# prachigarg23/MDIL-SS

Measured on AMD Instinct MI355X. Metric: images/sec at 1024x512 ERFNet-RA step-2 train (CS->BDD, KD on), batch 6/GPU, higher is better.
Workload: dtype f32; 1 GPU; ERFNet-RAP step-2 (2 student fwd + teacher fwd + CE + 0.1*KLD + bwd + Adam), random-init weights of the reference architecture, num_classes [20,20]; batch_per_gpu=6, global_batch=6, height=512, width=1024, parallelism=dp1

## Files before the change

### mdil_ss_amd/csrc/c16conv.hip

```cpp
#include "common.h"

namespace {

typedef unsigned int u32x4 __attribute__((ext_vector_type(4)));

constexpr int C16 = 16;
#ifndef C16_TN_
#define C16_TN_ 2
#endif
constexpr int C16_TN = C16_TN_;
constexpr int C16_PXT = 16 * C16_TN;
constexpr int C16_WAVES = 4;

struct c16_args {
  const float* in0;
  const float* in1;
  const float* wpk;
  float* out;
  mdil_epilogue e;
  int N, H, W;
  int ntaps;
  int dh[4], dw[4], src[4];
  int nwg;
};

__device__ __forceinline__ f32x4 c16_buf_load(const __amdgpu_buffer_rsrc_t r, unsigned voff) {
  const u32x4 v = __builtin_amdgcn_raw_buffer_load_b128(r, (int)voff, 0, 0);
  return __builtin_bit_cast(f32x4, v);
}

template <int NTAPS, bool EOPS>
__global__ __launch_bounds__(C16_WAVES * 64) void c16conv_kernel(const c16_args a) {
  const int lane = threadIdx.x & 63, wave = threadIdx.x >> 6;
  const int li = lane & 15, lg = lane >> 4;
  const int per = gridDim.x >> 3;
  const int g = (blockIdx.x & 7) * per + (blockIdx.x >> 3);
  if (g >= a.nwg) return;
  const int H = a.H, W = a.W, hw = H * W;
  const int npix = a.N * hw;
  const int tile = g * C16_WAVES + wave;
  const int P0 = tile * C16_PXT;
  if (P0 >= npix) return;

  const int in_bytes = npix * C16 * 4;
  const __amdgpu_buffer_rsrc_t rs0 =
      __builtin_amdgcn_make_buffer_rsrc(const_cast<float*>(a.in0), 0, in_bytes, 0x00020000);
  const __amdgpu_buffer_rsrc_t rs1 = __builtin_amdgcn_make_buffer_rsrc(
      const_cast<float*>(a.in1 ? a.in1 : a.in0), 0, in_bytes, 0x00020000);
  constexpr unsigned OOB = 0x80000000u;

  f32x4 xq[NTAPS][C16_TN];
  bool okp[C16_TN];
  long long pb[C16_TN];
#pragma unroll
  for (int n = 0; n < C16_TN; ++n) {
    const int P = P0 + 16 * n + li;
    okp[n] = P < npix;
    const int Pc = okp[n] ? P : 0;
    pb[n] = (long long)Pc * C16 + lg * 4;
    const int img = Pc / hw;
    const int rem = Pc - img * hw;
    const int h = rem / W;
    const int w = rem - h * W;
    const unsigned base = (unsigned)Pc * (unsigned)(C16 * 4) + (unsigned)lg * 16u;
#pragma unroll
    for (int t = 0; t < NTAPS; ++t) {
      const int hh = h + a.dh[t], ww = w + a.dw[t];
      const bool v = okp[n] && hh >= 0 && hh < H && ww >= 0 && ww < W;
      const unsigned voff = v ? base + (unsigned)((a.dh[t] * W + a.dw[t]) * C16 * 4) : OOB;
      xq[t][n] = c16_buf_load(a.src[t] ? rs1 : rs0, voff);
    }
  }
  const mdil_epilogue& e = a.e;
  f32x4 ra[C16_TN], rb[C16_TN];
  if constexpr (EOPS) {
    const float* opa = e.res ? e.res : e.gate;
    const float* opb = e.res_gate;
#pragma unroll
    for (int n = 0; n < C16_TN; ++n) {
      if (opa) ra[n] = *reinterpret_cast<const f32x4*>(opa + pb[n]);
      if (opb) rb[n] = *reinterpret_cast<const f32x4*>(opb + pb[n]);
    }
  }
  f32x4 wa[NTAPS];
#pragma unroll
  for (int t = 0; t < NTAPS; ++t) wa[t] = *reinterpret_cast<const f32x4*>(a.wpk + (t * C16 + li) * C16 + lg * 4);
  f32x4 vscale = {1.f, 1.f, 1.f, 1.f}, vbias = {0.f, 0.f, 0.f, 0.f};
  if (e.bias) vbias = *reinterpret_cast<const f32x4*>(e.bias + lg * 4);
  if (e.bias2) vbias += *reinterpret_cast<const f32x4*>(e.bias2 + lg * 4);
  if (e.scale) {
    vscale = *reinterpret_cast<const f32x4*>(e.scale + lg * 4);
    vbias = vbias * vscale + *reinterpret_cast<const f32x4*>(e.shift + lg * 4);
  }

  f32x4 acc[C16_TN];
#pragma unroll
  for (int n = 0; n < C16_TN; ++n) acc[n] = f32x4{0.f, 0.f, 0.f, 0.f};
#pragma unroll
  for (int t = 0; t < NTAPS; ++t)
#pragma unroll
    for (int s = 0; s < 4; ++s)
#pragma unroll
      for (int n = 0; n < C16_TN; ++n) acc[n] = mfma16(wa[t][s], xq[t][n][s], acc[n]);

#pragma unroll
  for (int n = 0; n < C16_TN; ++n) {
    f32x4 v = acc[n] * vscale + vbias;
    if (EOPS && e.res) {
      f32x4 x = ra[n];
      if (e.res_gate) {
#pragma unroll
        for (int k = 0; k < 4; ++k) x[k] = rb[n][k] > 0.f ? x[k] : 0.f;
      }
      v += x;
    }
    if (e.relu) {
#pragma unroll
      for (int k = 0; k < 4; ++k) v[k] = fmaxf(v[k], 0.f);
    }
    if (EOPS && e.gate && !e.res) {
#pragma unroll
      for (int k = 0; k < 4; ++k) v[k] = ra[n][k] > 0.f ? v[k] : 0.f;
    }
    if (okp[n]) __builtin_nontemporal_store(v, reinterpret_cast<f32x4*>(a.out + pb[n]));
  }
}

template <int NTAPS>
int launch_c16(const c16_args& a, hipStream_t st) {
  const int grid = (a.nwg + 7) / 8 * 8;
  const bool eops = a.e.res || a.e.gate || a.e.res_gate;
  if (eops)
    hipLaunchKernelGGL((c16conv_kernel<NTAPS, true>), dim3(grid), dim3(C16_WAVES * 64), 0, st, a);
  else
    hipLaunchKernelGGL((c16conv_kernel<NTAPS, false>), dim3(grid), dim3(C16_WAVES * 64), 0, st, a);
  MDIL_CHECK_LAUNCH();
  return MDIL_OK;
}

}

bool mdil_c16conv_covers(const mdil_geom* g, int cin, int cout, const mdil_epilogue* e) {
  if (cin != 16 || cout != 16 || g->ntaps != 3) return false;
  if (g->ihs != 1 || g->iws != 1 || g->ohs != 1 || g->ows != 1 || g->oho || g->owo ||
      g->HI != g->HO || g->WI != g->WO || g->OH != g->HO || g->OW != g->WO || g->out_coff ||
      g->out_pitch != 16 || g->in_pitch[0] != 16)
    return false;
  for (int t = 0; t < g->ntaps; ++t)
    if (g->src[t] && g->in_pitch[1] != 16) return false;
  if (e->res && e->gate) return false;
  return (long long)g->N * g->HO * g->WO * 16 * 4 < (1ll << 31);
}

int mdil_c16conv(const mdil_geom* g, const float* in0, const float* in1, const float* wpk,
                 const mdil_epilogue* epi, float* out, hipStream_t st) {
  c16_args a;
  memset(&a, 0, sizeof(a));
  a.in0 = in0;
  a.in1 = in1;
  a.wpk = wpk;
  a.out = out;
  a.e = *epi;
  a.N = g->N;
  a.H = g->HO;
  a.W = g->WO;
  a.ntaps = g->ntaps;
  for (int t = 0; t < g->ntaps; ++t) {
    a.dh[t] = g->dh[t];
    a.dw[t] = g->dw[t];
    a.src[t] = g->src[t];
  }
  const long long npix = (long long)g->N * g->HO * g->WO;
  const long long ntiles = (npix + C16_PXT - 1) / C16_PXT;
  a.nwg = (int)((ntiles + C16_WAVES - 1) / C16_WAVES);
  return launch_c16<3>(a, st);
}
```

### mdil_ss_amd/csrc/common.h

```cpp
#pragma once
#include <hip/hip_runtime.h>
#include <stdint.h>
#include <stdio.h>
#include <string.h>

#include "../../include/mdil_hip.h"

typedef float f32x4 __attribute__((ext_vector_type(4)));

#define MDIL_WG 256

#define MDIL_BN_MAX_BLOCKS 256

void mdil_set_error(const char* fmt, ...);

#define MDIL_CHECK_ARG(cond, ...)            \
  do {                                       \
    if (!(cond)) {                           \
      mdil_set_error(__VA_ARGS__);           \
      return MDIL_ERR_INVALID;               \
    }                                        \
  } while (0)

#define MDIL_CHECK_LAUNCH()                                              \
  do {                                                                   \
    hipError_t e__ = hipGetLastError();                                  \
    if (e__ != hipSuccess) {                                             \
      mdil_set_error("%s:%d launch failed: %s", __FILE__, __LINE__,      \
                     hipGetErrorString(e__));                            \
      return MDIL_ERR_LAUNCH;                                            \
    }                                                                    \
  } while (0)

#ifndef MDIL_HBM_PRIO
#define MDIL_HBM_PRIO 2
#endif
#define MDIL_HBM_KERNEL_PRIO() __builtin_amdgcn_s_setprio(MDIL_HBM_PRIO)

struct MdilProfScope {
  MdilProfScope(hipStream_t st, int kind, const mdil_geom* g, int cin, int cout);
  ~MdilProfScope();
  int idx;
  int path;
  hipStream_t st;
};

static inline int cdiv(long long a, long long b) { return (int)((a + b - 1) / b); }

__device__ __forceinline__ f32x4 mfma16(float a, float b, f32x4 c) {
  return __builtin_amdgcn_mfma_f32_16x16x4f32(a, b, c, 0, 0, 0);
}

__device__ __forceinline__ void welford_merge(float& n, float& mean, float& m2, float nb,
                                              float meanb, float m2b) {
  if (nb == 0.f) return;
  float nn = n + nb;
  float d = meanb - mean;
  float f = nb / nn;
  mean = mean + d * f;
  m2 = m2 + m2b + d * d * n * f;
  n = nn;
}

bool mdil_sconv_covers(const mdil_geom* g, int cin, int cout);
int mdil_sconv_stat_blocks(const mdil_geom* g, int cin);
int mdil_sconv(const mdil_geom* g, int cin, int cout, const float* in0, const float* in1,
               const float* wpk, const mdil_epilogue* epi, float* out, float* stats,
               float* stats_count, const float* bn_z, const float* bn_mean, const float* bn_invstd,
               hipStream_t st, const struct BnFinFwd* ff = nullptr, const struct BnFinBwd* fb = nullptr,
               int* fused = nullptr);

bool mdil_c16conv_covers(const mdil_geom* g, int cin, int cout, const mdil_epilogue* e);
int mdil_c16conv(const mdil_geom* g, const float* in0, const float* in1, const float* wpk,
                 const mdil_epilogue* epi, float* out, hipStream_t st);

bool mdil_wconv_covers(const mdil_geom* g, int cin, int cout);
int mdil_wconv_stat_blocks(const mdil_geom* g, int cin);
bool mdil_wconv_tail_covers(const mdil_geom* g);
struct BnFinFwd;
struct BnFinBwd;
int mdil_wconv(const mdil_geom* g, int cin, const float* in0, const float* in1, const float* wpk,
               const mdil_epilogue* epi, float* out, float* stats, float* stats_count,
               const float* bn_z, const float* bn_mean, const float* bn_invstd, hipStream_t st,
               const float* tail_gate = nullptr, const float* tail_drop = nullptr,
               const BnFinFwd* ff = nullptr, const BnFinBwd* fb = nullptr);

bool mdil_w4conv_covers(const mdil_geom* g, int cin, int cout);
int mdil_w4conv_stat_blocks(const mdil_geom* g, int cin);
int mdil_w4conv(const mdil_geom* g, int cin, const float* in0, const float* in1, const float* wpk,
                const mdil_epilogue* epi, float* out, float* stats, float* stats_count,
                const float* bn_z, const float* bn_mean, const float* bn_invstd, hipStream_t st,
                const float* tail_gate = nullptr, const float* tail_drop = nullptr,
                const BnFinFwd* ff = nullptr, const BnFinBwd* fb = nullptr);
static inline int mdil_wconv_form(const mdil_geom* g, int cin, int cout) {
  return mdil_w4conv_covers(g, cin, cout) ? 4 : mdil_wconv_covers(g, cin, cout) ? 2 : 0;
}

int mdil_bn_finalize_fwd(const float* partial, const float* pcount, int nblk, int C, const BnFinFwd& f,
                         hipStream_t st);
int mdil_bn_finalize_bwd(const float* partial, int nblk, int C, const BnFinBwd& f, hipStream_t st);
```

### mdil_ss_amd/csrc/errors.cpp

```cpp
#include <stdarg.h>
#include <stdio.h>

#include "../../include/mdil_hip.h"

static thread_local char g_err[512] = "";

void mdil_set_error(const char* fmt, ...) {
  va_list ap;
  va_start(ap, fmt);
  vsnprintf(g_err, sizeof(g_err), fmt, ap);
  va_end(ap);
}

extern "C" const char* mdil_last_error(void) { return g_err; }
extern "C" int mdil_version(void) { return 110; }
```

### mdil_ss_amd/csrc/tapconv.hip

```cpp
#include <stdlib.h>

#include <type_traits>

#include "common.h"
#include "bnfin.h"

#ifndef TC_TIMING
#define TC_TIMING 0
#endif
#if TC_TIMING
__device__ unsigned long long* tc_stamps = nullptr;
extern "C" int mdil_debug_set_stamps(void* p) {
  return (int)hipMemcpyToSymbol(HIP_SYMBOL(tc_stamps), &p, sizeof(p));
}
#define TC_STAMP(k)                                                             \
  do {                                                                          \
    if (threadIdx.x == 0 && tc_stamps) tc_stamps[blockIdx.x * 4 + (k)] = wall_clock64(); \
  } while (0)
#else
#define TC_STAMP(k)
#endif

namespace {

template <int CIN, int COUT, int BM_, bool STEM_>
struct TapCfg {
  static constexpr bool STEM = STEM_;
  static constexpr int BM = BM_;
  static constexpr int CIN_P = STEM ? 32 : ((CIN + 15) / 16 * 16);
#ifndef TC_KC_BIG
#define TC_KC_BIG 32
#endif
  static constexpr int KC = (CIN_P <= 48) ? CIN_P : TC_KC_BIG;
  static constexpr int NCHUNK = CIN_P / KC;
  static constexpr int QPR = KC / 4;
  static constexpr int LD = KC + 4;
  static constexpr int MT = (COUT + 15) / 16;
  static constexpr int COUT_P = MT * 16;
  static constexpr int NT = BM / 16;
  static constexpr bool SPLIT_CO = (MT % 4 == 0);
  static constexpr int TM = SPLIT_CO ? MT / 4 : MT;
  static constexpr int TN = SPLIT_CO ? NT : NT / 4;
  static constexpr int IN_ITEMS = BM * QPR / MDIL_WG;
  static constexpr int W_ITEMS = (COUT_P * QPR + MDIL_WG - 1) / MDIL_WG;
  static_assert(CIN_P % KC == 0, "chunking");
  static_assert((BM * QPR) % MDIL_WG == 0, "in-tile items");
  static_assert(SPLIT_CO || (NT % 4 == 0), "pixel tiles per wave");
};

template <int CIN, int COUT, int BM, bool STEM>
__global__ __launch_bounds__(MDIL_WG) void tapconv_kernel(const mdil_geom g,
                                                          const float* __restrict__ in0,
                                                          const float* __restrict__ in1,
                                                          const float* __restrict__ wpk,
                                                          const mdil_epilogue e,
                                                          float* __restrict__ out) {
  using C = TapCfg<CIN, COUT, BM, STEM>;
#ifndef TC_LDS_MIN
#define TC_LDS_MIN 0
#endif
  constexpr int SMEM_STAGE = (BM + C::COUT_P) * C::LD;
  constexpr int LDO = C::COUT_P + 4;
  constexpr int SMEM_OUT = (COUT % 4 == 0) ? BM * LDO + 2 * BM : 0;
  constexpr int SMEM_F = SMEM_STAGE > SMEM_OUT ? SMEM_STAGE : SMEM_OUT;
  __shared__ __attribute__((aligned(16))) float smem[SMEM_F > TC_LDS_MIN ? SMEM_F : TC_LDS_MIN];
  float* Is = smem;
  float* Ws = smem + BM * C::LD;

  const int tid = threadIdx.x;
  const int lane = tid & 63, wave = tid >> 6;
  const int li = lane & 15, lg = lane >> 4;
  const int npix = g.N * g.HO * g.WO;
  const int hw = g.HO * g.WO;
  const int tile0 = blockIdx.x * BM;

  int it_h[C::IN_ITEMS], it_w[C::IN_ITEMS];
  long long it_base[C::IN_ITEMS];
  if constexpr (!STEM) {
#pragma unroll
    for (int i = 0; i < C::IN_ITEMS; ++i) {
      const int idx = tid + MDIL_WG * i;
      const int p = idx / C::QPR;
      const int P = tile0 + p;
      if (P < npix) {
        const int n = P / hw;
        const int r = P - n * hw;
        const int ho = r / g.WO;
        const int wo = r - ho * g.WO;
        it_h[i] = ho * g.ihs;
        it_w[i] = wo * g.iws;
        it_base[i] = ((long long)n * g.HI + it_h[i]) * g.WI + it_w[i];
      } else {
        it_h[i] = -(1 << 28);
        it_w[i] = 0;
        it_base[i] = 0;
      }
    }
  }

#ifndef TC_PF2
#define TC_PF2 -1
#endif
  constexpr bool PF2 = TC_PF2 < 0 ? (C::CIN_P == 64) : (TC_PF2 != 0);
  constexpr int NSET = (PF2 && !STEM) ? 2 : 1;
  f32x4 regIs[NSET][C::IN_ITEMS];
  f32x4 regWs[NSET][C::W_ITEMS];
  unsigned okIs[NSET] = {};

  auto issue_loads = [&](auto SET, int t, int kc) {
    f32x4 (&regI)[C::IN_ITEMS] = regIs[decltype(SET)::value];
    f32x4 (&regW)[C::W_ITEMS] = regWs[decltype(SET)::value];
    unsigned& okI = okIs[decltype(SET)::value];
    if constexpr (!STEM) {
      const int s = g.src[t];
      const float* __restrict__ src = s ? in1 : in0;
      const int pitch = g.in_pitch[s];
      const int dh = g.dh[t], dw = g.dw[t];
      const long long tap_off = ((long long)dh * g.WI + dw) * pitch + kc * C::KC;
#pragma unroll
      for (int i = 0; i < C::IN_ITEMS; ++i) {
        const int idx = tid + MDIL_WG * i;
        const int q = idx % C::QPR;
        const int hi = it_h[i] + dh, wi = it_w[i] + dw;
        const int k = kc * C::KC + q * 4;
        const bool ok = (hi >= 0) && (hi < g.HI) && (wi >= 0) && (wi < g.WI) && (k < CIN);
        long long off = it_base[i] * pitch + (q * 4 + tap_off);
        off = ok ? off : 0ll;
        regI[i] = *reinterpret_cast<const f32x4*>(src + off);
        okI = ok ? (okI | (1u << i)) : (okI & ~(1u << i));
      }
    }
#pragma unroll
    for (int i = 0; i < C::W_ITEMS; ++i) {
      int idx = tid + MDIL_WG * i;
      if constexpr ((C::COUT_P * C::QPR) % MDIL_WG != 0) idx = idx < C::COUT_P * C::QPR ? idx : 0;
      const int co = idx / C::QPR, q = idx % C::QPR;
      regW[i] = *reinterpret_cast<const f32x4*>(wpk + ((long long)(t * C::COUT_P + co)) * C::CIN_P +
                                                kc * C::KC + q * 4);
    }
  };

  auto write_lds = [&](auto SET) {
    f32x4 (&regI)[C::IN_ITEMS] = regIs[decltype(SET)::value];
    f32x4 (&regW)[C::W_ITEMS] = regWs[decltype(SET)::value];
    const unsigned okI = okIs[decltype(SET)::value];
    if constexpr (!STEM) {
#pragma unroll
      for (int i = 0; i < C::IN_ITEMS; ++i) {
        const int idx = tid + MDIL_WG * i;
        const int p = idx / C::QPR, q = idx % C::QPR;
        const f32x4 z = {0.f, 0.f, 0.f, 0.f};
        *reinterpret_cast<f32x4*>(&Is[p * C::LD + q * 4]) = ((okI >> i) & 1u) ? regI[i] : z;
      }
    }
#pragma unroll
    for (int i = 0; i < C::W_ITEMS; ++i) {
      const int idx = tid + MDIL_WG * i;
      if (((C::COUT_P * C::QPR) % MDIL_WG == 0) || idx < C::COUT_P * C::QPR) {
        const int co = idx / C::QPR, q = idx % C::QPR;
        *reinterpret_cast<f32x4*>(&Ws[co * C::LD + q * 4]) = regW[i];
      }
    }
  };

  f32x4 acc[C::TM][C::TN];
#pragma unroll
  for (int a = 0; a < C::TM; ++a)
#pragma unroll
    for (int b = 0; b < C::TN; ++b) acc[a][b] = f32x4{0.f, 0.f, 0.f, 0.f};

  const int co_tile0 = C::SPLIT_CO ? wave * C::TM : 0;
  const int px_tile0 = C::SPLIT_CO ? 0 : wave * C::TN;

  if constexpr (STEM) {
    for (int idx = tid; idx < BM * 9; idx += MDIL_WG) {
      const int p = idx / 9, tap = idx - p * 9;
      const int P = tile0 + p;
      float v0 = 0.f, v1 = 0.f, v2 = 0.f;
      if (P < npix) {
        const int n = P / hw;
        const int r = P - n * hw;
        const int ho = r / g.WO, wo = r - (r / g.WO) * g.WO;
        const int hi = 2 * ho + tap / 3 - 1, wi = 2 * wo + tap % 3 - 1;
        if (hi >= 0 && hi < g.HI && wi >= 0 && wi < g.WI) {
          const float* s = in0 + ((long long)(n * g.HI + hi) * g.WI + wi) * 3;
          v0 = s[0];
          v1 = s[1];
          v2 = s[2];
        }
      }
      float* d = &Is[p * C::LD + 3 * tap];
      d[0] = v0;
      d[1] = v1;
      d[2] = v2;
    }
    for (int idx = tid; idx < BM * 5; idx += MDIL_WG) Is[(idx / 5) * C::LD + 27 + idx % 5] = 0.f;
  }

#ifndef TC_NT_STORE
#define TC_NT_STORE 1
#endif
#ifndef TC_ABLATE
#define TC_ABLATE 0
#endif
  const int nstage = g.ntaps * C::NCHUNK;
  using Set0 = std::integral_constant<int, 0>;
  using Set1 = std::integral_constant<int, NSET - 1>;
  TC_STAMP(0);
#if defined(TC_STAGGER) && TC_STAGGER > 0
  {
    const int slot = (blockIdx.x >> 8) % 3;
    for (int i = 0; i < slot * TC_STAGGER; ++i) __builtin_amdgcn_s_sleep(127);
  }
#endif
  auto mfma_stage = [&]() {
#ifndef TC_ROUND_UNROLL
#define TC_ROUND_UNROLL 1
#endif
#pragma unroll TC_ROUND_UNROLL
    for (int r = 0; r < C::KC / 16; ++r) {
      f32x4 a[C::TM], b[C::TN];
#pragma unroll
      for (int m = 0; m < C::TM; ++m)
        a[m] = *reinterpret_cast<const f32x4*>(&Ws[((co_tile0 + m) * 16 + li) * C::LD + r * 16 + lg * 4]);
#pragma unroll
      for (int n = 0; n < C::TN; ++n)
        b[n] = *reinterpret_cast<const f32x4*>(&Is[((px_tile0 + n) * 16 + li) * C::LD + r * 16 + lg * 4]);
#pragma unroll
      for (int s = 0; s < 4; ++s)
#pragma unroll
        for (int m = 0; m < C::TM; ++m)
#pragma unroll
          for (int n = 0; n < C::TN; ++n) acc[m][n] = mfma16(a[m][s], b[n][s], acc[m][n]);
    }
  };
  constexpr int DIST = NSET;
  auto stage = [&](auto SET, int st) {
    if (st == 1) TC_STAMP(1);
    if (TC_ABLATE < 2 || st == 0) {
      __syncthreads();
      write_lds(SET);
      __syncthreads();
    }
    if (st + DIST < nstage && (TC_ABLATE == 0)) {
      const int nx = st + DIST;
      issue_loads(SET, nx / C::NCHUNK, nx % C::NCHUNK);
    }
#ifndef TC_SETPRIO
#define TC_SETPRIO 1
#endif
#if TC_SETPRIO
    __builtin_amdgcn_s_setprio(1);
#endif
    mfma_stage();
#if TC_SETPRIO
    __builtin_amdgcn_s_setprio(0);
#endif
  };
  issue_loads(Set0{}, 0, 0);
  if constexpr (NSET == 2) {
    if (nstage > 1) issue_loads(Set1{}, 1 / C::NCHUNK, 1 % C::NCHUNK);
    for (int st = 0; st < nstage; st += 2) {
      stage(Set0{}, st);
      if (st + 1 < nstage) stage(Set1{}, st + 1);
    }
  } else {
    for (int st = 0; st < nstage; ++st) stage(Set0{}, st);
  }

  TC_STAMP(2);
  if constexpr (COUT % 4 == 0) {
    float* Os = smem;
    long long* Ob = reinterpret_cast<long long*>(smem + BM * LDO);
    constexpr bool QINV = (MDIL_WG % (COUT / 4)) == 0;
    f32x4 vscale = {1.f, 1.f, 1.f, 1.f}, vbias = {0.f, 0.f, 0.f, 0.f};
    if constexpr (QINV) {
      const int co0 = (tid % (COUT / 4)) * 4;
      if (e.bias) vbias = *reinterpret_cast<const f32x4*>(e.bias + co0);
      if (e.bias2) vbias += *reinterpret_cast<const f32x4*>(e.bias2 + co0);
      if (e.scale) {
        vscale = *reinterpret_cast<const f32x4*>(e.scale + co0);
        vbias = vbias * vscale + *reinterpret_cast<const f32x4*>(e.shift + co0);
      }
    }
    __syncthreads();
#pragma unroll
    for (int n = 0; n < C::TN; ++n)
#pragma unroll
      for (int m = 0; m < C::TM; ++m)
        *reinterpret_cast<f32x4*>(&Os[((px_tile0 + n) * 16 + li) * LDO + (co_tile0 + m) * 16 + lg * 4]) =
            acc[m][n];
    if (tid < BM) {
      const int P = tile0 + tid;
      long long ob = -1;
      if (P < npix) {
        const int ni = P / hw;
        const int r = P - ni * hw;
        const int ho = r / g.WO;
        const int wo = r - ho * g.WO;
        ob = ((long long)(ni * g.OH + ho * g.ohs + g.oho) * g.OW + (wo * g.ows + g.owo)) * g.out_pitch +
             g.out_coff;
      }
      Ob[tid] = ob;
    }
    __syncthreads();
    constexpr int QO = COUT / 4;
    constexpr int NIT = (BM * QO + MDIL_WG - 1) / MDIL_WG;
#pragma unroll
    for (int it = 0; it < NIT; ++it) {
      const int idx = tid + it * MDIL_WG;
      const bool in_tile = ((BM * QO) % MDIL_WG == 0) || idx < BM * QO;
      const int p = in_tile ? idx / QO : 0, q = idx % QO;
      const long long ob = Ob[p];
      const bool ok = in_tile && ob >= 0;
      const long long obase = ok ? ob : 0;
      const int co = q * 4;
      f32x4 v = *reinterpret_cast<const f32x4*>(&Os[p * LDO + co]);
      if constexpr (QINV) {
        v = v * vscale + vbias;
      } else {
        if (e.bias) v += *reinterpret_cast<const f32x4*>(e.bias + co);
        if (e.bias2) v += *reinterpret_cast<const f32x4*>(e.bias2 + co);
        if (e.scale)
          v = v * *reinterpret_cast<const f32x4*>(e.scale + co) +
              *reinterpret_cast<const f32x4*>(e.shift + co);
      }
      if (e.res) {
        f32x4 rr = *reinterpret_cast<const f32x4*>(e.res + obase + co);
        if (e.res_gate) {
          const f32x4 gg = *reinterpret_cast<const f32x4*>(e.res_gate + obase + co);
#pragma unroll
          for (int k = 0; k < 4; ++k) rr[k] = gg[k] > 0.f ? rr[k] : 0.f;
        }
        v += rr;
      }
      if (e.relu) {
#pragma unroll
        for (int k = 0; k < 4; ++k) v[k] = fmaxf(v[k], 0.f);
      }
      if (e.gate) {
        const f32x4 gg = *reinterpret_cast<const f32x4*>(e.gate + obase + co);
#pragma unroll
        for (int k = 0; k < 4; ++k) v[k] = gg[k] > 0.f ? v[k] : 0.f;
      }
      if (ok) {
#if TC_NT_STORE
        __builtin_nontemporal_store(v, reinterpret_cast<f32x4*>(out + obase + co));
#else
        *reinterpret_cast<f32x4*>(out + obase + co) = v;
#endif
      }
    }
  } else {
#pragma unroll
    for (int n = 0; n < C::TN; ++n) {
      const int P = tile0 + (px_tile0 + n) * 16 + li;
      if (P >= npix) continue;
      const int ni = P / hw;
      const int r = P - ni * hw;
      const int ho = r / g.WO;
      const int wo = r - ho * g.WO;
      const long long obase =
          ((long long)(ni * g.OH + ho * g.ohs + g.oho) * g.OW + (wo * g.ows + g.owo)) * g.out_pitch +
          g.out_coff;
#pragma unroll
      for (int m = 0; m < C::TM; ++m) {
        const int co = (co_tile0 + m) * 16 + lg * 4;
        const f32x4 v = acc[m][n];
#pragma unroll
        for (int k = 0; k < 4; ++k) {
          const int c = co + k;
          if (c >= COUT) continue;
          float x = v[k];
          if (e.bias) x += e.bias[c];
          if (e.bias2) x += e.bias2[c];
          if (e.scale) x = x * e.scale[c] + e.shift[c];
          if (e.res) {
            float rr = e.res[obase + c];
            if (e.res_gate) rr = e.res_gate[obase + c] > 0.f ? rr : 0.f;
            x += rr;
          }
          if (e.relu) x = fmaxf(x, 0.f);
          if (e.gate) x = e.gate[obase + c] > 0.f ? x : 0.f;
          out[obase + c] = x;
        }
      }
    }
  }
#if TC_TIMING
  asm volatile("s_waitcnt vmcnt(0)" ::: "memory");
  TC_STAMP(3);
#endif
}

__device__ __forceinline__ void pack_one(const mdil_pack_job& j, int first, int step) {
  const int total = j.ntaps * j.M_P * j.K_P;
  for (int idx = first; idx < total; idx += step) {
    const int k = idx % j.K_P;
    const int m = (idx / j.K_P) % j.M_P;
    const int t = idx / (j.K_P * j.M_P);
    float v = 0.f;
    if (m < j.M && k < j.K) {
      const long long off = j.stem ? (long long)m * 27 + (k % 3) * 9 + k / 3
                                   : (long long)m * j.s_m + (long long)k * j.s_k + j.ktap[t];
      v = j.src[off];
    }
    j.dst[idx] = v;
  }
}

__global__ void pack_weights_kernel(const mdil_pack_job j) {
  pack_one(j, blockIdx.x * blockDim.x + threadIdx.x, gridDim.x * blockDim.x);
}

__global__ void pack_weights_batch_kernel(const mdil_pack_job* __restrict__ jobs) {
  const mdil_pack_job j = jobs[blockIdx.x];
  pack_one(j, blockIdx.y * blockDim.x + threadIdx.x, gridDim.y * blockDim.x);
}

template <int CIN, int COUT, int BM, bool STEM>
int launch_tapconv(const mdil_geom* g, const float* in0, const float* in1, const float* wpk,
                   const mdil_epilogue* epi, float* out, hipStream_t st) {
  const long long npix = (long long)g->N * g->HO * g->WO;
  const int grid = cdiv(npix, BM);
  hipLaunchKernelGGL((tapconv_kernel<CIN, COUT, BM, STEM>), dim3(grid), dim3(MDIL_WG), 0, st, *g,
                     in0, in1, wpk, *epi, out);
  MDIL_CHECK_LAUNCH();
  return MDIL_OK;
}

}

extern "C" int mdil_pack_weights(const float* src, float* dst, int ntaps, const int* ktap, int M,
                                 int K, int M_P, int K_P, int s_m, int s_k, int stem, void* stream) {
  MDIL_CHECK_ARG(ntaps >= 1 && ntaps <= MDIL_MAX_TAPS, "pack_weights: ntaps=%d", ntaps);
  MDIL_CHECK_ARG(M_P >= M && K_P >= K, "pack_weights: padded dims smaller than dims");
  mdil_pack_job j;
  memset(&j, 0, sizeof(j));
  j.src = src;
  j.dst = dst;
  j.ntaps = ntaps;
  j.M = M;
  j.K = K;
  j.M_P = M_P;
  j.K_P = K_P;
  j.s_m = s_m;
  j.s_k = s_k;
  j.stem = stem;
  for (int t = 0; t < ntaps; ++t) j.ktap[t] = ktap ? ktap[t] : 0;
  const int total = ntaps * M_P * K_P;
  hipLaunchKernelGGL(pack_weights_kernel, dim3(cdiv(total, 256) > 1024 ? 1024 : cdiv(total, 256)),
                     dim3(256), 0, (hipStream_t)stream, j);
  MDIL_CHECK_LAUNCH();
  return MDIL_OK;
}

extern "C" int mdil_pack_weights_batch(const mdil_pack_job* jobs_device, int njobs, void* stream) {
  MDIL_CHECK_ARG(jobs_device && njobs >= 0, "pack_weights_batch: bad argument");
  if (njobs == 0) return MDIL_OK;
  hipLaunchKernelGGL(pack_weights_batch_kernel, dim3(njobs, 16), dim3(256), 0, (hipStream_t)stream,
                     jobs_device);
  MDIL_CHECK_LAUNCH();
  return MDIL_OK;
}

static int conv_path(const mdil_geom* g, int cin, int cout) {
  const int form = mdil_wconv_form(g, cin, cout);
  return form == 4 ? 4 : form == 2 ? 2 : 1;
}

extern "C" int mdil_tapconv_stat_blocks(const mdil_geom* g, int cin, int cout) {
  static const bool use_sconv = getenv("MDIL_NO_SCONV") == nullptr && getenv("MDIL_NO_BNFUSE") == nullptr;
  if (!g || !use_sconv || !mdil_sconv_covers(g, cin, cout)) return 0;
  return mdil_sconv_stat_blocks(g, cin);
}

extern "C" int mdil_tapconv_stats(const mdil_geom* g, int cin, int cout, const float* in0,
                                  const float* in1, const float* wpk, const mdil_epilogue* epi,
                                  float* out, float* partial, float* pcount, void* stream) {
  MDIL_CHECK_ARG(g && epi && in0 && wpk && out && partial && pcount, "tapconv_stats: null argument");
  MDIL_CHECK_ARG(mdil_tapconv_stat_blocks(g, cin, cout) > 0, "tapconv_stats: call cannot emit statistics");
  MDIL_CHECK_ARG((epi->scale == nullptr) == (epi->shift == nullptr), "tapconv_stats: scale/shift");
  MdilProfScope ps((hipStream_t)stream, 0, g, cin, cout);
  ps.path = conv_path(g, cin, cout);
  return mdil_sconv(g, cin, cout, in0, in1, wpk, epi, out, partial, pcount, nullptr, nullptr, nullptr,
                    (hipStream_t)stream);
}

static BnFinBwd make_fin_bwd(const mdil_bn_grad* fin, const float* save_invstd, long long npix) {
  BnFinBwd f;
  memset(&f, 0, sizeof(f));
  if (fin && fin->coef) {
    f.ticket = fin->ticket;
    f.gamma = fin->gamma, f.save_invstd = save_invstd;
    f.dgamma = fin->dgamma, f.dbeta = fin->dbeta, f.accumulate = fin->accumulate;
    f.n = (float)npix;
    f.coef = fin->coef;
  }
  return f;
}

extern "C" int mdil_tapconv_bnred(const mdil_geom* g, int cin, int cout, const float* in0,
                                  const float* in1, const float* wpk, const mdil_epilogue* epi,
                                  float* out, const float* bn_z, const float* save_mean,
                                  const float* save_invstd, float* partial, const mdil_bn_grad* fin,
                                  void* stream) {
  MDIL_CHECK_ARG(g && epi && in0 && wpk && out && bn_z && save_mean && save_invstd && partial,
                 "tapconv_bnred: null argument");
  const int nblk = mdil_tapconv_stat_blocks(g, cin, cout);
  MDIL_CHECK_ARG(nblk > 0, "tapconv_bnred: call is not covered");
  MDIL_CHECK_ARG(!epi->res_gate && !(epi->res && epi->gate), "tapconv_bnred: epilogue combination");
  MDIL_CHECK_ARG(!fin || (fin->gamma && fin->coef), "tapconv_bnred: fin needs gamma and coef");
  const BnFinBwd fb = make_fin_bwd(fin, save_invstd, (long long)g->N * g->HO * g->WO);
  int fused = 0;
  {
    MdilProfScope ps((hipStream_t)stream, 0, g, cin, cout);
    ps.path = conv_path(g, cin, cout);
    const int rc = mdil_sconv(g, cin, cout, in0, in1, wpk, epi, out, partial, nullptr, bn_z, save_mean,
                              save_invstd, (hipStream_t)stream, nullptr, fin ? &fb : nullptr, &fused);
    if (rc) return rc;
  }
  if (fin && !fused) {
    BnFinBwd f = fb;
    f.ticket = nullptr;
    return mdil_bn_finalize_bwd(partial, nblk, cout, f, (hipStream_t)stream);
  }
  return MDIL_OK;
}

extern "C" int mdil_tapconv_bn_train(const mdil_geom* g, int cin, int cout, const float* in0,
                                     const float* in1, const float* wpk, const mdil_epilogue* epi,
                                     float* out, const mdil_bn_train* bn, void* workspace,
                                     size_t workspace_bytes, unsigned int* ticket, void* stream) {
  MDIL_CHECK_ARG(g && epi && in0 && wpk && out && bn, "tapconv_bn_train: null argument");
  MDIL_CHECK_ARG(bn->gamma && bn->beta && bn->coef, "tapconv_bn_train: BatchNorm fields");
  const long long npix = (long long)g->N * g->HO * g->WO;
  MDIL_CHECK_ARG(workspace && workspace_bytes >= mdil_bn_workspace(npix, cout), "tapconv_bn_train: workspace");
  float* c = bn->coef;
  const int nblk = mdil_tapconv_stat_blocks(g, cin, cout);
  if (nblk == 0 || epi->scale) {
    const int rc = mdil_tapconv(g, cin, cout, in0, in1, wpk, epi, out, stream);
    if (rc) return rc;
    return mdil_bn_train_stats(out, npix, cout, bn->gamma, bn->beta, bn->running_mean, bn->running_var,
                               bn->num_batches_tracked, bn->eps, bn->momentum, c, c + cout, c + 2 * cout,
                               c + 3 * cout, workspace, workspace_bytes, ticket, stream);
  }
  float* partial = (float*)workspace;
  float* pcount = partial + (size_t)MDIL_BN_MAX_BLOCKS * 2 * cout;
  BnFinFwd ff;
  ff.ticket = ticket;
  ff.gamma = bn->gamma, ff.beta = bn->beta;
  ff.running_mean = bn->running_mean, ff.running_var = bn->running_var, ff.nbt = bn->num_batches_tracked;
  ff.eps = bn->eps, ff.momentum = bn->momentum;
  ff.save_mean = c, ff.save_invstd = c + cout, ff.scale = c + 2 * cout, ff.shift = c + 3 * cout;
  int fused = 0;
  {
    MdilProfScope ps((hipStream_t)stream, 0, g, cin, cout);
    ps.path = conv_path(g, cin, cout);
    const int rc = mdil_sconv(g, cin, cout, in0, in1, wpk, epi, out, partial, pcount, nullptr, nullptr,
                              nullptr, (hipStream_t)stream, &ff, nullptr, &fused);
    if (rc) return rc;
  }
  if (fused) return MDIL_OK;
  ff.ticket = nullptr;
  return mdil_bn_finalize_fwd(partial, pcount, nblk, cout, ff, (hipStream_t)stream);
}

extern "C" int mdil_tapconv_tail_blocks(const mdil_geom* g, int cin, int cout) {
  static const bool on = getenv("MDIL_NO_SCONV") == nullptr && getenv("MDIL_NO_BNFUSE") == nullptr &&
                         getenv("MDIL_NO_BNTAIL") == nullptr;
  if (!g || !on || !mdil_sconv_covers(g, cin, cout) || !mdil_wconv_covers(g, cin, cout) ||
      !mdil_wconv_tail_covers(g))
    return 0;
  return mdil_wconv_stat_blocks(g, cin);
}

extern "C" int mdil_tapconv_tail(const mdil_geom* g, int cin, int cout, const float* in0,
                                 const float* in1, const float* wpk, const mdil_epilogue* epi,
                                 float* out, const mdil_bn_tail* t, void* stream) {
  MDIL_CHECK_ARG(g && epi && in0 && wpk && out && t, "tapconv_tail: null argument");
  MDIL_CHECK_ARG(t->gate && t->z && t->save_mean && t->save_invstd && t->partial, "tapconv_tail: tail fields");
  MDIL_CHECK_ARG(mdil_tapconv_tail_blocks(g, cin, cout) > 0, "tapconv_tail: call is not covered");
  MDIL_CHECK_ARG(!epi->gate && !epi->relu && !epi->scale && (epi->res || !epi->res_gate),
                 "tapconv_tail: epilogue combination");
  for (int k = 0; k < g->ntaps; ++k)
    MDIL_CHECK_ARG(g->src[k] == 0 || (g->src[k] == 1 && in1), "tapconv_tail: tap %d source", k);
  MDIL_CHECK_ARG(!t->fin.coef || t->fin.gamma, "tapconv_tail: fin needs gamma");
  const BnFinBwd fb = make_fin_bwd(&t->fin, t->save_invstd, (long long)g->N * g->HO * g->WO);
  {
    MdilProfScope ps((hipStream_t)stream, 0, g, cin, cout);
    ps.path = conv_path(g, cin, cout);
    const int rc = mdil_wconv(g, cin, in0, in1, wpk, epi, out, t->partial, nullptr, t->z, t->save_mean,
                              t->save_invstd, (hipStream_t)stream, t->gate, t->drop, nullptr,
                              t->fin.coef ? &fb : nullptr);
    if (rc) return rc;
  }
  if (t->fin.coef && !t->fin.ticket)
    return mdil_bn_finalize_bwd(t->partial, mdil_tapconv_tail_blocks(g, cin, cout), cout, fb, (hipStream_t)stream);
  return MDIL_OK;
}

extern "C" int mdil_tapconv(const mdil_geom* g, int cin, int cout, const float* in0,
                            const float* in1, const float* wpk, const mdil_epilogue* epi,
                            float* out, void* stream) {
  MDIL_CHECK_ARG(g && epi && in0 && wpk && out, "tapconv: null argument");
  MDIL_CHECK_ARG(g->ntaps >= 1 && g->ntaps <= MDIL_MAX_TAPS, "tapconv: ntaps=%d", g->ntaps);
  MDIL_CHECK_ARG((long long)g->N * g->HO * g->WO < (1ll << 31), "tapconv: grid too large");
  MDIL_CHECK_ARG((epi->scale == nullptr) == (epi->shift == nullptr), "tapconv: scale/shift");
  for (int t = 0; t < g->ntaps; ++t) {
    MDIL_CHECK_ARG(g->src[t] == 0 || (g->src[t] == 1 && in1), "tapconv: tap %d source", t);
    MDIL_CHECK_ARG((cin == 27 && cout == 13) || g->in_pitch[g->src[t]] % 4 == 0, "tapconv: pitch %% 4");
  }
  hipStream_t st = (hipStream_t)stream;
  MdilProfScope ps(st, 0, g, cin, cout);
  static const bool use_sconv = getenv("MDIL_NO_SCONV") == nullptr;
  if (use_sconv) {
    const int rc = mdil_sconv(g, cin, cout, in0, in1, wpk, epi, out, nullptr, nullptr, nullptr, nullptr,
                              nullptr, st);
    if (rc != MDIL_ERR_UNSUPPORTED) {
      ps.path = conv_path(g, cin, cout);
      return rc;
    }
  }
  static const bool use_c16 = getenv("MDIL_NO_C16CONV") == nullptr;
  if (use_c16 && mdil_c16conv_covers(g, cin, cout, epi)) {
    ps.path = 3;
    return mdil_c16conv(g, in0, in1, wpk, epi, out, st);
  }
#define TC(ci, co, bm, stem) \
  if (cin == ci && cout == co) return launch_tapconv<ci, co, bm, stem>(g, in0, in1, wpk, epi, out, st)
  TC(64, 64, 128, false);
  TC(128, 128, 64, false);
  TC(16, 16, 128, false);
  TC(16, 48, 128, false);
  TC(48, 16, 128, false);
  TC(128, 64, 128, false);
  TC(64, 128, 64, false);
  TC(64, 16, 128, false);
  TC(16, 64, 128, false);
  TC(16, 20, 128, false);
  TC(20, 16, 128, false);
  TC(16, 27, 128, false);
  TC(27, 16, 128, false);
  TC(27, 13, 128, true);
#undef TC
  mdil_set_error("tapconv: no tile configuration for cin=%d cout=%d", cin, cout);
  return MDIL_ERR_UNSUPPORTED;
}
```

Baseline: 270.3 images/sec.

## Fuse BatchNorm statistics and finalize into 16-channel MFMA conv kernel

Adds a persistent 16-wave variant of the 16x16-channel 3-tap MFMA convolution. It accumulates per-channel Welford statistics in the forward pass, or the BN-backward reductions (sum and sum times centered input) in the backward pass. The last block finalizes them through a ticket, and the next tile's loads are double-buffered to overlap with compute. Tapconv routes 16-channel BN-fused calls to this kernel instead of the generic sconv path, removing separate stats or finalize passes and a slower generic kernel. In exchange it runs a persistent grid capped at the CU count, which may reduce occupancy.

```diff
diff --git a/mdil_ss_amd/csrc/c16conv.hip b/mdil_ss_amd/csrc/c16conv.hip
--- a/mdil_ss_amd/csrc/c16conv.hip
+++ b/mdil_ss_amd/csrc/c16conv.hip
@@ -1,4 +1,8 @@
+#include <stdlib.h>
+
 #include "common.h"
+#include "bnfin.h"
+#include "wino.h"
 
 namespace {
 
@@ -126,6 +130,255 @@
   }
 }
 
+constexpr int C16F_WAVES = 16;
+constexpr int C16F_SW = 36;
+
+struct c16f_args {
+  c16_args c;
+  int ntiles;
+  float* stats;
+  float* stats_count;
+  const float* bn_z;
+  const float* bn_mean;
+  const float* bn_invstd;
+  BnFinFwd ff;
+  BnFinBwd fb;
+};
+
+struct c16_tile {
+  f32x4 xq[3][C16_TN];
+  unsigned pb[C16_TN];
+  bool ok[C16_TN];
+};
+
+template <int MODE, bool EOPS>
+__global__ __launch_bounds__(C16F_WAVES * 64) void c16fuse_kernel(const c16f_args fa) {
+  constexpr int NTAPS = 3;
+  constexpr bool BNRED = MODE == 2;
+  __shared__ float Sw[C16F_WAVES * C16F_SW];
+  __shared__ __attribute__((aligned(16))) double Fs[2 * 8 * C16];
+  __shared__ int flag;
+  const c16_args& a = fa.c;
+  const int lane = threadIdx.x & 63, wave = threadIdx.x >> 6;
+  const int li = lane & 15, lg = lane >> 4;
+  const int H = a.H, W = a.W, hw = H * W;
+  const int npix = a.N * hw;
+  const int per = gridDim.x >> 3;
+  const int xcd = blockIdx.x & 7;
+  const int tpx = (fa.ntiles + 7) >> 3;
+  const int t_last = (xcd + 1) * tpx < fa.ntiles ? (xcd + 1) * tpx : fa.ntiles;
+  const int stride = per * C16F_WAVES;
+  const int tile0 = xcd * tpx + (blockIdx.x >> 3) * C16F_WAVES + wave;
+
+  const int in_bytes = npix * C16 * 4;
+  const __amdgpu_buffer_rsrc_t rs0 =
+      __builtin_amdgcn_make_buffer_rsrc(const_cast<float*>(a.in0), 0, in_bytes, 0x00020000);
+  const __amdgpu_buffer_rsrc_t rs1 = __builtin_amdgcn_make_buffer_rsrc(
+      const_cast<float*>(a.in1 ? a.in1 : a.in0), 0, in_bytes, 0x00020000);
+  constexpr unsigned OOB = 0x80000000u;
+
+  auto issue = [&](c16_tile& T, int tile) __attribute__((always_inline)) {
+    const int P0 = tile * C16_PXT;
+#pragma unroll
+    for (int n = 0; n < C16_TN; ++n) {
+      const int P = P0 + 16 * n + li;
+      T.ok[n] = P < npix;
+      const int Pc = T.ok[n] ? P : 0;
+      T.pb[n] = (unsigned)Pc * C16 + lg * 4;
+      const int img = Pc / hw;
+      const int rem = Pc - img * hw;
+      const int h = rem / W;
+      const int w = rem - h * W;
+      const unsigned base = (unsigned)Pc * (unsigned)(C16 * 4) + (unsigned)lg * 16u;
+#pragma unroll
+      for (int t = 0; t < NTAPS; ++t) {
+        const int hh = h + a.dh[t], ww = w + a.dw[t];
+        const bool v = T.ok[n] && hh >= 0 && hh < H && ww >= 0 && ww < W;
+        const unsigned voff = v ? base + (unsigned)((a.dh[t] * W + a.dw[t]) * C16 * 4) : OOB;
+        T.xq[t][n] = c16_buf_load(a.src[t] ? rs1 : rs0, voff);
+      }
+    }
+  };
+
+  const mdil_epilogue& e = a.e;
+  f32x4 wa[NTAPS];
+#pragma unroll
+  for (int t = 0; t < NTAPS; ++t) wa[t] = *reinterpret_cast<const f32x4*>(a.wpk + (t * C16 + li) * C16 + lg * 4);
+  f32x4 vscale = {1.f, 1.f, 1.f, 1.f}, vbias = {0.f, 0.f, 0.f, 0.f};
+  if constexpr (!BNRED) {
+    if (e.bias) vbias = *reinterpret_cast<const f32x4*>(e.bias + lg * 4);
+    if (e.bias2) vbias += *reinterpret_cast<const f32x4*>(e.bias2 + lg * 4);
+    if (e.scale) {
+      vscale = *reinterpret_cast<const f32x4*>(e.scale + lg * 4);
+      vbias = vbias * vscale + *reinterpret_cast<const f32x4*>(e.shift + lg * 4);
+    }
+  }
+  f32x4 mu = {0.f, 0.f, 0.f, 0.f};
+  if constexpr (BNRED) mu = *reinterpret_cast<const f32x4*>(fa.bn_mean + lg * 4);
+
+  float sn = 0.f;
+  f32x4 sA = {0.f, 0.f, 0.f, 0.f}, sB = {0.f, 0.f, 0.f, 0.f};
+
+  auto step = [&](c16_tile& T, c16_tile& Tn, int next) __attribute__((always_inline)) {
+    f32x4 ra[C16_TN], rb[C16_TN];
+    if constexpr (EOPS) {
+      const float* opa = e.res ? e.res : e.gate;
+      const float* opb = BNRED ? nullptr : e.res_gate;
+#pragma unroll
+      for (int n = 0; n < C16_TN; ++n) {
+        if (opa) ra[n] = *reinterpret_cast<const f32x4*>(opa + T.pb[n]);
+        if (opb) rb[n] = *reinterpret_cast<const f32x4*>(opb + T.pb[n]);
+      }
+    }
+    if constexpr (BNRED) {
+#pragma unroll
+      for (int n = 0; n < C16_TN; ++n) rb[n] = *reinterpret_cast<const f32x4*>(fa.bn_z + T.pb[n]);
+    }
+    if (next < t_last) issue(Tn, next);
+
+    f32x4 acc[C16_TN];
+#pragma unroll
+    for (int n = 0; n < C16_TN; ++n) acc[n] = f32x4{0.f, 0.f, 0.f, 0.f};
+#pragma unroll
+    for (int t = 0; t < NTAPS; ++t)
+#pragma unroll
+      for (int s = 0; s < 4; ++s)
+#pragma unroll
+        for (int n = 0; n < C16_TN; ++n) acc[n] = mfma16(wa[t][s], T.xq[t][n][s], acc[n]);
+
+#pragma unroll
+    for (int n = 0; n < C16_TN; ++n) {
+      f32x4 v = acc[n];
+      if constexpr (!BNRED) v = acc[n] * vscale + vbias;
+      if (EOPS && e.res) {
+        f32x4 x = ra[n];
+        if (!BNRED && e.res_gate) {
+#pragma unroll
+          for (int k = 0; k < 4; ++k) x[k] = rb[n][k] > 0.f ? x[k] : 0.f;
+        }
+        v += x;
+      }
+      if (e.relu) {
+#pragma unroll
+        for (int k = 0; k < 4; ++k) v[k] = fmaxf(v[k], 0.f);
+      }
+      if (EOPS && e.gate && !e.res) {
+#pragma unroll
+        for (int k = 0; k < 4; ++k) v[k] = ra[n][k] > 0.f ? v[k] : 0.f;
+      }
+      if (T.ok[n]) __builtin_nontemporal_store(v, reinterpret_cast<f32x4*>(a.out + T.pb[n]));
+      if constexpr (BNRED) {
+        const f32x4 z = {0.f, 0.f, 0.f, 0.f};
+        const f32x4 gv = T.ok[n] ? v : z;
+        sA += gv;
+        sB += gv * (rb[n] - mu);
+      } else {
+        const float nn = sn + (T.ok[n] ? 1.f : 0.f);
+        const float f = T.ok[n] ? __builtin_amdgcn_rcpf(nn) : 0.f;
+        const float nf = sn * f;
+        const f32x4 d = v - sA;
+        sA += d * f;
+        sB += (d * d) * nf;
+        sn = nn;
+      }
+    }
+  };
+
+  {
+    c16_tile TA, TB;
+    int tile = tile0;
+    if (tile < t_last) issue(TA, tile);
+    while (tile < t_last) {
+      step(TA, TB, tile + stride);
+      tile += stride;
+      if (tile >= t_last) break;
+      step(TB, TA, tile + stride);
+      tile += stride;
+    }
+  }
+
+#pragma unroll
+  for (int off = 8; off >= 1; off >>= 1) {
+    if constexpr (BNRED) {
+#pragma unroll
+      for (int k = 0; k < 4; ++k) {
+        sA[k] += __shfl_xor(sA[k], off);
+        sB[k] += __shfl_xor(sB[k], off);
+      }
+    } else {
+      const float on = __shfl_xor(sn, off);
+      float nk = sn;
+#pragma unroll
+      for (int k = 0; k < 4; ++k) {
+        const float om = __shfl_xor(sA[k], off), oq = __shfl_xor(sB[k], off);
+        nk = sn;
+        float mk = sA[k], qk = sB[k];
+        welford_merge(nk, mk, qk, on, om, oq);
+        sA[k] = mk;
+        sB[k] = qk;
+      }
+      sn = nk;
+    }
+  }
+  float* mine = Sw + wave * C16F_SW;
+  if (li == 0) {
+#pragma unroll
+    for (int k = 0; k < 4; ++k) {
+      mine[lg * 4 + k] = sA[k];
+      mine[C16 + lg * 4 + k] = sB[k];
+    }
+  }
+  if (lane == 0) mine[2 * C16] = sn;
+  __syncthreads();
+  const int row = blockIdx.x, nrows = gridDim.x;
+  const int tid = threadIdx.x;
+  if constexpr (BNRED) {
+    if (tid < C16) {
+      float sa = 0.f, sb = 0.f;
+#pragma unroll
+      for (int w = 0; w < C16F_WAVES; ++w) {
+        sa += Sw[w * C16F_SW + tid];
+        sb += Sw[w * C16F_SW + C16 + tid];
+      }
+      sb *= fa.bn_invstd[tid];
+      float* r0 = fa.stats + ((long long)row * 2 + 0) * C16 + tid;
+      float* r1 = fa.stats + ((long long)row * 2 + 1) * C16 + tid;
+      if (fa.fb.ticket) {
+        bnfin_st(r0, sa);
+        bnfin_st(r1, sb);
+      } else {
+        *r0 = sa;
+        *r1 = sb;
+      }
+    }
+    if (fa.fb.ticket) {
+      if (bnfin_arrive(fa.fb.ticket, nrows, &flag)) bnfin_backward(fa.fb, fa.stats, nrows, C16, Fs);
+    }
+  } else {
+    if (tid < C16) {
+      float n = 0.f, mean = 0.f, m2 = 0.f;
+#pragma unroll
+      for (int w = 0; w < C16F_WAVES; ++w)
+        welford_merge(n, mean, m2, Sw[w * C16F_SW + 2 * C16], Sw[w * C16F_SW + tid], Sw[w * C16F_SW + C16 + tid]);
+      float* r0 = fa.stats + ((long long)row * 2 + 0) * C16 + tid;
+      float* r1 = fa.stats + ((long long)row * 2 + 1) * C16 + tid;
+      if (fa.ff.ticket) {
+        bnfin_st(r0, mean);
+        bnfin_st(r1, m2);
+        if (tid == 0) bnfin_st(fa.stats_count + row, n);
+      } else {
+        *r0 = mean;
+        *r1 = m2;
+        if (tid == 0) fa.stats_count[row] = n;
+      }
+    }
+    if (fa.ff.ticket) {
+      if (bnfin_arrive(fa.ff.ticket, nrows, &flag))
+        bnfin_forward(fa.ff, fa.stats, fa.stats_count, nrows, C16, reinterpret_cast<float*>(Fs));
+    }
+  }
+}
+
 template <int NTAPS>
 int launch_c16(const c16_args& a, hipStream_t st) {
   const int grid = (a.nwg + 7) / 8 * 8;
@@ -152,9 +405,8 @@
   return (long long)g->N * g->HO * g->WO * 16 * 4 < (1ll << 31);
 }
 
-int mdil_c16conv(const mdil_geom* g, const float* in0, const float* in1, const float* wpk,
-                 const mdil_epilogue* epi, float* out, hipStream_t st) {
-  c16_args a;
+static void c16_fill(c16_args& a, const mdil_geom* g, const float* in0, const float* in1, const float* wpk,
+                     const mdil_epilogue* epi, float* out) {
   memset(&a, 0, sizeof(a));
   a.in0 = in0;
   a.in1 = in1;
@@ -170,8 +422,64 @@
     a.dw[t] = g->dw[t];
     a.src[t] = g->src[t];
   }
+}
+
+int mdil_c16conv(const mdil_geom* g, const float* in0, const float* in1, const float* wpk,
+                 const mdil_epilogue* epi, float* out, hipStream_t st) {
+  c16_args a;
+  c16_fill(a, g, in0, in1, wpk, epi, out);
   const long long npix = (long long)g->N * g->HO * g->WO;
   const long long ntiles = (npix + C16_PXT - 1) / C16_PXT;
   a.nwg = (int)((ntiles + C16_WAVES - 1) / C16_WAVES);
   return launch_c16<3>(a, st);
 }
+
+int mdil_c16conv_stat_blocks(const mdil_geom* g) {
+  const long long npix = (long long)g->N * g->HO * g->WO;
+  const long long ntiles = (npix + C16_PXT - 1) / C16_PXT;
+  long long nq = (ntiles + C16F_WAVES - 1) / C16F_WAVES;
+  if (nq > wc_num_cu()) nq = wc_num_cu();
+  nq = (nq + 7) / 8 * 8;
+  return (int)(nq > MDIL_BN_MAX_BLOCKS ? MDIL_BN_MAX_BLOCKS : nq);
+}
+
+int mdil_c16conv_fused(const mdil_geom* g, const float* in0, const float* in1, const float* wpk,
+                       const mdil_epilogue* epi, float* out, float* stats, float* stats_count,
+                       const float* bn_z, const float* bn_mean, const float* bn_invstd, hipStream_t st,
+                       const BnFinFwd* ff, const BnFinBwd* fb, int* fused) {
+  if (fused) *fused = 0;
+  if (!mdil_c16conv_covers(g, 16, 16, epi)) return MDIL_ERR_UNSUPPORTED;
+  if (!stats || (!bn_z && !stats_count) || (bn_z && (!bn_mean || !bn_invstd || epi->res_gate)))
+    return MDIL_ERR_INVALID;
+  if (bn_z && (epi->bias || epi->bias2 || epi->scale || epi->shift)) return MDIL_ERR_INVALID;
+  c16f_args fa;
+  memset(&fa, 0, sizeof(fa));
+  c16_fill(fa.c, g, in0, in1, wpk, epi, out);
+  const long long npix = (long long)g->N * g->HO * g->WO;
+  fa.ntiles = (int)((npix + C16_PXT - 1) / C16_PXT);
+  fa.stats = stats;
+  fa.stats_count = stats_count;
+  fa.bn_z = bn_z;
+  fa.bn_mean = bn_mean;
+  fa.bn_invstd = bn_invstd;
+  if (ff && !bn_z) fa.ff = *ff;
+  if (fb && bn_z) fa.fb = *fb;
+  const int grid = mdil_c16conv_stat_blocks(g);
+  const bool eops = epi->res || epi->gate || epi->res_gate;
+  const dim3 blk(C16F_WAVES * 64);
+  if (bn_z) {
+    if (eops)
+      hipLaunchKernelGGL((c16fuse_kernel<2, true>), dim3(grid), blk, 0, st, fa);
+    else
+      hipLaunchKernelGGL((c16fuse_kernel<2, false>), dim3(grid), blk, 0, st, fa);
+    if (fused) *fused = fa.fb.ticket != nullptr;
+  } else {
+    if (eops)
+      hipLaunchKernelGGL((c16fuse_kernel<1, true>), dim3(grid), blk, 0, st, fa);
+    else
+      hipLaunchKernelGGL((c16fuse_kernel<1, false>), dim3(grid), blk, 0, st, fa);
+    if (fused) *fused = fa.ff.ticket != nullptr;
+  }
+  MDIL_CHECK_LAUNCH();
+  return MDIL_OK;
+}
diff --git a/mdil_ss_amd/csrc/common.h b/mdil_ss_amd/csrc/common.h
--- a/mdil_ss_amd/csrc/common.h
+++ b/mdil_ss_amd/csrc/common.h
@@ -73,6 +73,12 @@
 bool mdil_c16conv_covers(const mdil_geom* g, int cin, int cout, const mdil_epilogue* e);
 int mdil_c16conv(const mdil_geom* g, const float* in0, const float* in1, const float* wpk,
                  const mdil_epilogue* epi, float* out, hipStream_t st);
+int mdil_c16conv_stat_blocks(const mdil_geom* g);
+int mdil_c16conv_fused(const mdil_geom* g, const float* in0, const float* in1, const float* wpk,
+                       const mdil_epilogue* epi, float* out, float* stats, float* stats_count,
+                       const float* bn_z, const float* bn_mean, const float* bn_invstd, hipStream_t st,
+                       const struct BnFinFwd* ff = nullptr, const struct BnFinBwd* fb = nullptr,
+                       int* fused = nullptr);
 
 bool mdil_wconv_covers(const mdil_geom* g, int cin, int cout);
 int mdil_wconv_stat_blocks(const mdil_geom* g, int cin);
diff --git a/mdil_ss_amd/csrc/errors.cpp b/mdil_ss_amd/csrc/errors.cpp
--- a/mdil_ss_amd/csrc/errors.cpp
+++ b/mdil_ss_amd/csrc/errors.cpp
@@ -13,4 +13,4 @@
 }
 
 extern "C" const char* mdil_last_error(void) { return g_err; }
-extern "C" int mdil_version(void) { return 110; }
+extern "C" int mdil_version(void) { return 111; }
diff --git a/mdil_ss_amd/csrc/tapconv.hip b/mdil_ss_amd/csrc/tapconv.hip
--- a/mdil_ss_amd/csrc/tapconv.hip
+++ b/mdil_ss_amd/csrc/tapconv.hip
@@ -469,9 +469,20 @@
   return form == 4 ? 4 : form == 2 ? 2 : 1;
 }
 
+static bool c16_fused_form(const mdil_geom* g, int cin, int cout) {
+  static const bool on = getenv("MDIL_NO_C16CONV") == nullptr && getenv("MDIL_NO_BNFUSE") == nullptr &&
+                         getenv("MDIL_NO_C16BNFUSE") == nullptr;
+  if (!on) return false;
+  mdil_epilogue none;
+  memset(&none, 0, sizeof(none));
+  return mdil_c16conv_covers(g, cin, cout, &none);
+}
+
 extern "C" int mdil_tapconv_stat_blocks(const mdil_geom* g, int cin, int cout) {
   static const bool use_sconv = getenv("MDIL_NO_SCONV") == nullptr && getenv("MDIL_NO_BNFUSE") == nullptr;
-  if (!g || !use_sconv || !mdil_sconv_covers(g, cin, cout)) return 0;
+  if (!g) return 0;
+  if (c16_fused_form(g, cin, cout)) return mdil_c16conv_stat_blocks(g);
+  if (!use_sconv || !mdil_sconv_covers(g, cin, cout)) return 0;
   return mdil_sconv_stat_blocks(g, cin);
 }
 
@@ -482,6 +493,12 @@
   MDIL_CHECK_ARG(mdil_tapconv_stat_blocks(g, cin, cout) > 0, "tapconv_stats: call cannot emit statistics");
   MDIL_CHECK_ARG((epi->scale == nullptr) == (epi->shift == nullptr), "tapconv_stats: scale/shift");
   MdilProfScope ps((hipStream_t)stream, 0, g, cin, cout);
+  if (c16_fused_form(g, cin, cout)) {
+    MDIL_CHECK_ARG(mdil_c16conv_covers(g, cin, cout, epi), "tapconv_stats: epilogue combination");
+    ps.path = 3;
+    return mdil_c16conv_fused(g, in0, in1, wpk, epi, out, partial, pcount, nullptr, nullptr, nullptr,
+                              (hipStream_t)stream);
+  }
   ps.path = conv_path(g, cin, cout);
   return mdil_sconv(g, cin, cout, in0, in1, wpk, epi, out, partial, pcount, nullptr, nullptr, nullptr,
                     (hipStream_t)stream);
@@ -515,9 +532,13 @@
   int fused = 0;
   {
     MdilProfScope ps((hipStream_t)stream, 0, g, cin, cout);
-    ps.path = conv_path(g, cin, cout);
-    const int rc = mdil_sconv(g, cin, cout, in0, in1, wpk, epi, out, partial, nullptr, bn_z, save_mean,
-                              save_invstd, (hipStream_t)stream, nullptr, fin ? &fb : nullptr, &fused);
+    const bool c16 = c16_fused_form(g, cin, cout);
+    ps.path = c16 ? 3 : conv_path(g, cin, cout);
+    const int rc = c16 ? mdil_c16conv_fused(g, in0, in1, wpk, epi, out, partial, nullptr, bn_z, save_mean,
+                                            save_invstd, (hipStream_t)stream, nullptr, fin ? &fb : nullptr,
+                                            &fused)
+                       : mdil_sconv(g, cin, cout, in0, in1, wpk, epi, out, partial, nullptr, bn_z, save_mean,
+                                    save_invstd, (hipStream_t)stream, nullptr, fin ? &fb : nullptr, &fused);
     if (rc) return rc;
   }
   if (fin && !fused) {
@@ -538,7 +559,8 @@
   MDIL_CHECK_ARG(workspace && workspace_bytes >= mdil_bn_workspace(npix, cout), "tapconv_bn_train: workspace");
   float* c = bn->coef;
   const int nblk = mdil_tapconv_stat_blocks(g, cin, cout);
-  if (nblk == 0 || epi->scale) {
+  const bool c16 = nblk > 0 && c16_fused_form(g, cin, cout);
+  if (nblk == 0 || epi->scale || (c16 && !mdil_c16conv_covers(g, cin, cout, epi))) {
     const int rc = mdil_tapconv(g, cin, cout, in0, in1, wpk, epi, out, stream);
     if (rc) return rc;
     return mdil_bn_train_stats(out, npix, cout, bn->gamma, bn->beta, bn->running_mean, bn->running_var,
@@ -556,9 +578,11 @@
   int fused = 0;
   {
     MdilProfScope ps((hipStream_t)stream, 0, g, cin, cout);
-    ps.path = conv_path(g, cin, cout);
-    const int rc = mdil_sconv(g, cin, cout, in0, in1, wpk, epi, out, partial, pcount, nullptr, nullptr,
-                              nullptr, (hipStream_t)stream, &ff, nullptr, &fused);
+    ps.path = c16 ? 3 : conv_path(g, cin, cout);
+    const int rc = c16 ? mdil_c16conv_fused(g, in0, in1, wpk, epi, out, partial, pcount, nullptr, nullptr,
+                                            nullptr, (hipStream_t)stream, &ff, nullptr, &fused)
+                       : mdil_sconv(g, cin, cout, in0, in1, wpk, epi, out, partial, pcount, nullptr, nullptr,
+                                    nullptr, (hipStream_t)stream, &ff, nullptr, &fused);
     if (rc) return rc;
   }
   if (fused) return MDIL_OK;
```

New measurement: 272.0 images/sec, median of 6. About the same (+0.6%).
